# PKU-EPIC/HOTrack

Measured on AMD Instinct MI355X. Metric: HandTrackNet point-cloud frames/sec (N=1024), higher is better.
Workload: dtype f32; 1 GPU; HandTrackNet forward, batch=64 synthetic 1024-pt clouds per GPU (BASELINE configs[1]); per_gpu_batch=64, global_batch=64, npoints=1024, parallelism=dp1 (independent batches, no collective), world_size=1, resident_batches_rotated=5, dead_attention_elided=True, fused_sa_kernels=True, launch=hipGraph replay, batches_in_flight=4, hip_hw_queues=4, sa_compute_units=256, weights=deterministic random init (no checkpoint available offline)

## Files before the change

### hotrack_amd/csrc/row_chain.hip

```cpp
#include "pn2_common.h"
#include "../../include/pn2_ext.h"

namespace pn2 {
namespace rchain {

typedef float f32x4 __attribute__((ext_vector_type(4)));

constexpr int CH = 128, CC = 384, CQ = 512;
constexpr int KX = 144;
constexpr int XQ = 33;
constexpr int LDX = 152, LDH = 136, LDC = 392;
constexpr int MAXB = 1024;
constexpr int GROUP_COST_SMALL = 31, GROUP_COST_LARGE = 20;

struct ChainArgs {
    int B, N, ldx, ldo;
    const float *x;
    const int *list, *counts;
    const float *wa, *ba, *wb, *bb, *wc, *bc, *wq;
    float *out;
};

template <int NT, int MT, int KG, int LD>
__device__ __forceinline__ void mm(f32x4 (&acc)[NT][MT], const float *__restrict__ wp, const float *xs, int lane) {
    const f32x4 *w4 = reinterpret_cast<const f32x4 *>(wp) + lane;
    const float *xr = xs + (lane & 15) * LD + 4 * (lane >> 4);
    f32x4 w[2][NT], x[2][MT];
    auto load = [&](int kg, int slot) {
#pragma unroll
        for (int nt = 0; nt < NT; ++nt) w[slot][nt] = w4[(nt * KG + kg) * 64];
#pragma unroll
        for (int mt = 0; mt < MT; ++mt) x[slot][mt] = *reinterpret_cast<const f32x4 *>(xr + mt * 16 * LD + 16 * kg);
    };
    auto step = [&](int slot) {
#pragma unroll
        for (int s = 0; s < 4; ++s)
#pragma unroll
            for (int nt = 0; nt < NT; ++nt)
#pragma unroll
                for (int mt = 0; mt < MT; ++mt)
                    acc[nt][mt] = __builtin_amdgcn_mfma_f32_16x16x4f32(w[slot][nt][s], x[slot][mt][s], acc[nt][mt], 0, 0, 0);
    };
    load(0, 0);
    int kg = 0;
#pragma unroll 1
    for (; kg + 2 <= KG; kg += 2) {
        load(kg + 1, 1);
        step(0);
        if (kg + 2 < KG) load(kg + 2, 0);
        step(1);
    }
    if constexpr (KG & 1) step(0);
}

template <int NT, int MT>
__device__ __forceinline__ void init_bias(f32x4 (&acc)[NT][MT], const float *__restrict__ bias, int nt0, int lane) {
#pragma unroll
    for (int nt = 0; nt < NT; ++nt) {
        const f32x4 b = *reinterpret_cast<const f32x4 *>(bias + (nt0 + nt) * 16 + 4 * (lane >> 4));
#pragma unroll
        for (int mt = 0; mt < MT; ++mt) acc[nt][mt] = b;
    }
}

template <int NT, int MT>
__device__ __forceinline__ void relu_to_lds(const f32x4 (&acc)[NT][MT], float *dst, int ld, int nt0, int lane) {
#pragma unroll
    for (int nt = 0; nt < NT; ++nt)
#pragma unroll
        for (int mt = 0; mt < MT; ++mt) {
            const f32x4 v = acc[nt][mt];
            *reinterpret_cast<f32x4 *>(dst + (mt * 16 + (lane & 15)) * ld + (nt0 + nt) * 16 + 4 * (lane >> 4)) =
                (f32x4){fmaxf(v.x, 0.f), fmaxf(v.y, 0.f), fmaxf(v.z, 0.f), fmaxf(v.w, 0.f)};
        }
}

struct Smem {
    int *rows;
    int *p_small;
    int *p_large;
    float *r1;
    float *r2;
};

__device__ __forceinline__ int lookup(const ChainArgs &A, const Smem &S, int seq, int e) {
    const int *P = seq ? S.p_large : S.p_small;
    int lo = 0, hi = A.B;
    while (hi - lo > 1) {
        const int mid = (lo + hi) >> 1;
        if (P[mid] <= e) lo = mid; else hi = mid;
    }
    const int off = seq ? (S.p_small[lo + 1] - S.p_small[lo]) : 0;
    return lo * A.N + A.list[(size_t)lo * A.N + off + (e - P[lo])];
}

template <int MT>
__device__ void tile(const ChainArgs &A, const Smem &S, int seq, int e0, int cnt) {
    const int tid = (int)threadIdx.x, lane = tid & 63, w = tid >> 6;
    constexpr int R = MT * 16;
    if (tid < R) S.rows[tid] = tid < cnt ? lookup(A, S, seq, e0 + tid) : -1;
    __syncthreads();
    for (int i = tid; i < R * (KX / 4); i += 256) {
        const int r = i / (KX / 4), q = i - r * (KX / 4);
        const int g = S.rows[r];
        f32x4 v = {0.f, 0.f, 0.f, 0.f};
        if (g >= 0 && q < XQ) {
            v = *reinterpret_cast<const f32x4 *>(A.x + (size_t)g * A.ldx + 4 * q);
            if (q == XQ - 1) v.w = 0.f;
        }
        *reinterpret_cast<f32x4 *>(S.r1 + r * LDX + 4 * q) = v;
    }
    __syncthreads();
    {
        f32x4 acc[2][MT];
        init_bias(acc, A.ba, 2 * w, lane);
        mm<2, MT, KX / 16, LDX>(acc, A.wa + (size_t)(2 * w) * (KX / 16) * 256, S.r1, lane);
        relu_to_lds(acc, S.r2, LDH, 2 * w, lane);
    }
    __syncthreads();
    {
        f32x4 acc[2][MT];
        init_bias(acc, A.bb, 2 * w, lane);
        mm<2, MT, CH / 16, LDH>(acc, A.wb + (size_t)(2 * w) * (CH / 16) * 256, S.r2, lane);
        relu_to_lds(acc, S.r1, LDH, 2 * w, lane);
    }
    __syncthreads();
#pragma unroll 1
    for (int p = 0; p < 2; ++p) {
// ... 185 lines not shown
```

### hotrack_amd/ext.py

```python
from __future__ import annotations

import ctypes
import os

import torch

from . import pointnet2_hip as _native

_lib = _native._lib
_vp, _ci = ctypes.c_void_p, ctypes.c_int
_lib.pn2x_kabsch.argtypes = [_ci, _ci, _ci, _vp, _vp, _vp, _vp, _vp]
_lib.pn2x_kabsch.restype = _ci


def kabsch(x: torch.Tensor, y: torch.Tensor):
    x = x.float().contiguous()
    y = y.float().contiguous()
    if x.dim() == 2:
        x = x.unsqueeze(0)
    B, num, _ = y.shape
    xb = x.shape[0]
    if xb not in (1, B) or x.shape[1] != num:
        raise ValueError(f"kabsch: x {tuple(x.shape)} does not match y {tuple(y.shape)}")
    px = _native._ptr(x, "x", torch.float32, xb * num * 3)
# ... 616 lines not shown


def row_lists(gi: torch.Tensor, gi_small, n: int):
    if gi.dim() != 3 or gi.dtype != torch.int32 or not gi.is_cuda:
        raise TypeError("row_lists: gi must be a (B,J,K) int32 GPU tensor")
    gi = gi.contiguous()
    B, J, KL = gi.shape
    if gi_small is not None:
        if gi_small.dim() != 3 or gi_small.shape[:2] != (B, J) or gi_small.dtype != torch.int32 or gi_small.device != gi.device:
            raise ValueError("row_lists: gi_small must be (B,J,K2) int32 on gi's device")
        gi_small = gi_small.contiguous()
    KS = gi_small.shape[2] if gi_small is not None else KL
    lst = torch.empty((B, n), dtype=torch.int32, device=gi.device)
    counts = torch.empty((B, 2), dtype=torch.int32, device=gi.device)
    with torch.cuda.device(gi.device):
        _native._check(_native._call(_lib.pn2x_row_lists, "row_lists_kernel", None, B, n, J, KL, KS, gi.data_ptr(),
                                     None if gi_small is None else gi_small.data_ptr(), lst.data_ptr(), counts.data_ptr(),
                                     _native._stream(gi)), "row_lists")
    return lst, counts


def row_chain_supported(c_in: int, c_h: int, c_conv: int, c_q: int) -> bool:
    return bool(_lib.pn2x_row_chain_supported(c_in, c_h, c_conv, c_q))


def row_chain_pack(W: torch.Tensor) -> torch.Tensor:
    n_out, k = W.shape
    kp = (k + 15) // 16 * 16
    Wp = torch.zeros((n_out, kp), dtype=torch.float32, device=W.device)
    Wp[:, :k] = W
    return Wp.view(n_out // 16, 16, kp // 16, 4, 4).permute(0, 2, 3, 1, 4).contiguous()


def row_chain(x: torch.Tensor, lst: torch.Tensor, counts: torch.Tensor, wa, ba, wb, bb, wc, bc, wq, out: torch.Tensor = None,
              grid: int = 0) -> torch.Tensor:
    if x.dim() != 3 or not x.is_cuda or x.dtype != torch.float32 or x.stride(2) != 1 or x.stride(0) != x.shape[1] * x.stride(1):
        raise TypeError("row_chain: x must be a (B,N,C) float32 GPU tensor with contiguous rows")
    B, N, _ = x.shape
    f32 = torch.float32
    if out is None:
        out = torch.empty((B, N, 512), dtype=f32, device=x.device)
    if out.shape[:2] != (B, N) or out.shape[2] < 512 or out.stride(2) != 1 or out.stride(0) != N * out.stride(1) or out.dtype != f32:
        raise ValueError("row_chain: out must be (B,N,>=512) float32 with contiguous rows")
    if lst.shape != (B, N) or counts.shape != (B, 2) or lst.dtype != torch.int32 or counts.dtype != torch.int32:
        raise ValueError("row_chain: list (B,N) / counts (B,2) int32 from row_lists")
    with torch.cuda.device(x.device):
        _native._check(_native._call(_lib.pn2x_row_chain, "row_chain_kernel", None, B, N, x.data_ptr(), x.stride(1), lst.data_ptr(),
                                     counts.data_ptr(), _native._ptr(wa, "wa", f32, 128 * 144), _native._ptr(ba, "ba", f32, 128),
                                     _native._ptr(wb, "wb", f32, 128 * 128), _native._ptr(bb, "bb", f32, 128),
                                     _native._ptr(wc, "wc", f32, 384 * 128), _native._ptr(bc, "bc", f32, 384),
                                     _native._ptr(wq, "wq", f32, 512 * 384), out.data_ptr(), out.stride(1), int(grid),
                                     _native._stream(x)), "row_chain")
    return out
```

### include/pn2_ext.h

```cpp
#ifndef PN2_EXT_H
#define PN2_EXT_H

#include "pn2_hip.h"

#ifdef __cplusplus
extern "C" {
#endif

int pn2x_kabsch(int b, int xb, int num, const float *x, const float *y, float *R, float *t, void *stream);
int pn2x_kabsch_backward(int b, int xb, int num, const float *x, const float *y, const float *R, const float *grad_R,
                         const float *grad_t, float *grad_y, void *stream);

int pn2x_hand_frame(int b, int xb, int num, int n, int j, const float *palm_template, const float *kp,
                    const int *palm_idx, const float *points, float scale, float *R, float *t, float *xyz2,
                    float *xyz1, float *xyz2_copy, int copy_ld, int *nonfinite, void *stream);

int pn2x_sa_mlp_max(int b, int n, int s, int k, int c1, int c2, int c3, const float *a1f, int a1f_ld,
                    const float *xyz, const float *cxyz, const float *wx, const float *b1, const float *cadd,
                    int cadd_ld, const int *idx,
                    const float *w2, const float *b2, const float *w3, const float *b3, float *out,
                    long out_b, int out_s, int out_c, void *stream);
int pn2x_sa_mlp_max_supported(int k, int c1, int c2, int c3);

int pn2x_bias_act(int b, int c, int n, float *y, const float *bias, int relu, void *stream);
// ... 18 lines not shown
int pn2x_fps_prefix_flags(int n);
int pn2x_furthest_point_sampling_prefix(int b, int n, int m, const float *xyz, const int *flags, int nflags, int *idx, void *stream);

int pn2x_knn_indices(int b, int n, int m, int k, int k2, const float *unknown, const float *known, int *idx, int *idx2, void *stream);

int pn2x_ball_query_picks(int b, int n, int m, float radius, int nsample, const float *xyz, const int *picks, float *new_xyz,
                          int *idx, float *new_xyz_copy, int copy_ld, void *stream);

long pn2x_ball_query_grid_scratch_words(int b, int n);
int pn2x_ball_query_grid(int b, int n, int m, float radius, int nsample, const float *new_xyz, const float *xyz, int *idx,
                         void *scratch, long scratch_words, void *stream);

int pn2x_gather_rows(int b, int n, int m, int c, const float *src, const int *idx, float *out, void *stream);

int pn2x_bias_act_pm(long rows, int c, float *y, int ldy, const float *bias, long rows_per_bias, int relu, void *stream);

int pn2x_max_rows(int b, int r, int c, const float *x, float *out, void *stream);

int pn2x_copy_multi_max(void);
int pn2x_copy_multi(int n, void *const *dst, const void *const *src, const long *bytes, void *stream);

int pn2x_add_layernorm(long rows, int c, const float *x, const float *y, const float *bias, const float *g1,
                       const float *b1, float eps1, const float *g2, const float *b2, float eps2, float *out, void *stream);

int pn2x_pose_head(int b, int j, int c, const float *h, const float *w, const float *bias, const float *xyz1,
                   const float *R, const float *t, float scale, float *kp_hand, float *kp_cam, const int *nonfinite,
                   void *stream);

typedef struct pn2x_sa_problem {
    int n, s, k;
    const float *a1f;
    int a1f_ld;
    const float *xyz, *cxyz, *wx, *b1, *cadd;
    int cadd_ld;
    const int *idx;
    const float *w2, *b2, *w3, *b3;
    float *out;
    long out_b;
    int out_s, out_c;
} pn2x_sa_problem;
int pn2x_sa_set_compute_units(int n);
int pn2x_mlp2_rows_supported(int c1, int c2, int c3);
int pn2x_mlp2_rows(long rows, int c1, int c2, int c3, const float *x, int ldx, const float *w2, const float *w2e, const float *b2,
                   const float *w3, const float *b3, float *out, int ldo, void *stream);
int pn2x_sa_mlp_max_pair_supported(int k0, int k1, int c1, int c2, int c3);
int pn2x_sa_mlp_max_pair(int b, int c1, int c2, int c3, const pn2x_sa_problem *p0, const pn2x_sa_problem *p1, void *stream);

int pn2x_row_lists(int b, int n, int j, int k_large, int k_small, const int *gi, const int *gi_small, int *list, int *counts,
                   void *stream);
int pn2x_row_chain_supported(int c_in, int c_h, int c_conv, int c_q);
int pn2x_row_chain(int b, int n, const float *x, int ldx, const int *list, const int *counts, const float *wa, const float *ba,
                   const float *wb, const float *bb, const float *wc, const float *bc, const float *wq, float *out, int ldo,
                   int grid, void *stream);

int pn2x_bn_sums_doubles(int c);
int pn2x_bn_stats(long rows, int c, const float *y, int ldy, double *sums, void *stream);
int pn2x_bn_relu_apply(long rows, int c, const float *y, int ldy, const double *sums, const float *gamma, const float *beta,
                       const float *conv_bias, float eps, float momentum, float *running_mean, float *running_var,
                       long long *num_batches_tracked, float *save_mean, float *save_invstd, float *h, int ldh, int relu,
                       void *stream);
int pn2x_bn_relu_bwd(long rows, int c, const float *dh, int ldd, const float *y, int ldy, const float *mean,
                     const float *invstd, const float *gamma, const float *beta, int relu, double *sums, float *dy, int ldo,
                     float *dgamma, float *dbeta, float *dbias, void *stream);
int pn2x_sa_layer1(int b, int n, int s, int k, int c1, const float *a1f, int a1f_ld, const float *xyz, const float *cxyz,
                   const float *wx, int wx_ld, const float *cadd, int cadd_ld, const int *idx, float *out, float *rel_out,
                   void *stream);
int pn2x_sa_layer1_stats(int b, int n, int s, int k, int c1, const float *a1f, int a1f_ld, const float *xyz, const float *cxyz,
                         const float *wx, int wx_ld, const float *cadd, int cadd_ld, const int *idx, float *out, float *rel_out,
                         double *sums, void *stream);
int pn2x_sa_layer1_stats_pair(int b, int n, int s, const float *xyz, const float *cxyz, int k_a, int c1_a, const float *a1f_a, int a1f_ld_a,
                              const float *wx_a, int wx_ld_a, const float *cadd_a, int cadd_ld_a, const int *idx_a, float *out_a,
                              float *rel_out_a, double *sums_a, int k_b, int c1_b, const float *a1f_b, int a1f_ld_b, const float *wx_b,
                              int wx_ld_b, const float *cadd_b, int cadd_ld_b, const int *idx_b, float *out_b, float *rel_out_b,
                              double *sums_b, void *stream);
int pn2x_scatter_add_rows(int b, int n, int m, int c, const float *dout, int ldo, const int *idx, float *din, int ldi,
                          void *stream);
int pn2x_three_interpolate_pm_grad(int b, int c, int m, int n, const float *dout, int ldo, const int *idx,
                                   const float *weight, float *dpoints, int ldp, void *stream);

int pn2x_inverse_index(int b, int n_dst, int l, const int *idx, int *offsets, int *order, void *stream);
int pn2x_rows_segment_sum(int b, int n_dst, int m_src, int t, int c, const float *dout, int ldo, const int *offsets,
                          const int *order, const float *weight, float *din, int ldi, int accumulate, void *stream);
int pn2x_rows_segment_sum_pair(int b, int n_dst, int m_a, int c_a, const float *dout_a, int ldo_a, const int *offsets_a, const int *order_a,
                               float *din_a, int ldi_a, int m_b, int c_b, const float *dout_b, int ldo_b, const int *offsets_b,
                               const int *order_b, float *din_b, int ldi_b, int accumulate, void *stream);

long pn2x_scatter_cm_scratch_ints(int t, int b, int n_dst, int m_src);
int pn2x_scatter_cm(int t, int b, int c, int n_dst, int m_src, const float *grad_out, const int *idx, const float *weight,
                    float *grad_points, int *scratch, long scratch_ints, void *stream);

int pn2x_bn_relu_max(long groups, int k, int c, const float *y, int ldy, const double *sums, const float *gamma, const float *beta,
                     const float *conv_bias, float eps, float momentum, float *running_mean, float *running_var,
                     long long *num_batches_tracked, float *save_mean, float *save_invstd, float *out, int *arg, void *stream);
int pn2x_bn_relu_max_ld(long groups, int k, int c, const float *y, int ldy, const double *sums, const float *gamma, const float *beta,
                        const float *conv_bias, float eps, float momentum, float *running_mean, float *running_var,
                        long long *num_batches_tracked, float *save_mean, float *save_invstd, float *out, int ldo, int *arg, void *stream);
int pn2x_bn_relu_max_pair(long groups_a, int k_a, int c_a, const float *y_a, int ldy_a, const double *sums_a, const float *gamma_a,
                          const float *beta_a, const float *conv_bias_a, float eps_a, float momentum_a, float *running_mean_a,
                          float *running_var_a, long long *nbt_a, float *save_mean_a, float *save_invstd_a, float *out_a, int ldo_a,
                          int *arg_a, long groups_b, int k_b, int c_b, const float *y_b, int ldy_b, const double *sums_b,
                          const float *gamma_b, const float *beta_b, const float *conv_bias_b, float eps_b, float momentum_b,
                          float *running_mean_b, float *running_var_b, long long *nbt_b, float *save_mean_b, float *save_invstd_b,
                          float *out_b, int ldo_b, int *arg_b, void *stream);
int pn2x_bn_relu_max_bwd(long groups, int k, int c, const float *dout, const int *arg, const float *y, int ldy, const float *mean,
                         const float *invstd, const float *gamma, const float *beta, double *sums, float *dy, int ldo, float *dgamma,
                         float *dbeta, float *dbias, void *stream);
// ... 126 lines not shown
```

### network/models/fast_eval.py

```python
from __future__ import annotations

import torch
import torch.nn.functional as F



def _lin_relu(x2d: torch.Tensor, W: torch.Tensor, b: torch.Tensor) -> torch.Tensor:
    from hotrack_amd import ext
    return ext.linear(x2d, W, b, relu=True)


def _lin(x2d: torch.Tensor, W: torch.Tensor, b: torch.Tensor = None) -> torch.Tensor:
    from hotrack_amd import ext
    return ext.linear(x2d, W, b)


class FastEval:
    MAX_POINTS = 16384

    def __init__(self, net):
        self.net = net
        self._shapes_seen = set()
        self._key = None
        self.P = None
# ... 57 lines not shown
        gemm_tuning.enable()
        net, bh = self.net, self.net.bhand
        P = {}

        def msg(mod, i):
            return [fold(c, n) for c, n in zip(mod.conv_blocks[i], mod.bn_blocks[i])]

        (W1, b1), l2, l3 = msg(bh.sa1, 0)
        P["sa1"] = dict(wx=W1.contiguous(), b1=b1, l2=l2, l3=l3)
        (W1, b1), l2, l3 = msg(bh.sa2, 0)
        D = W1.shape[1] - 3
        P["sa2"] = dict(w1f=W1[:, :D].contiguous(), wx=W1[:, D:].contiguous(), b1=b1, l2=l2, l3=l3)
        sa3 = [fold(c, n) for c, n in zip(bh.sa3.mlp_convs, bh.sa3.mlp_bns)]
        W = sa3[0][0]
        sa3[0] = (torch.cat([W[:, 3:], W[:, :3]], dim=1).contiguous(), sa3[0][1])
        P["sa3"] = sa3
        fp3 = [fold(c, n) for c, n in zip(bh.fp3.mlp_convs, bh.fp3.mlp_bns)]
        c_l2 = bh.sa2.out_channel
        P["fp3"] = dict(wa=fp3[0][0][:, :c_l2].contiguous(), wb=fp3[0][0][:, c_l2:].contiguous(), b=fp3[0][1], rest=fp3[1:])
        P["fp2"] = [fold(c, n) for c, n in zip(bh.fp2.mlp_convs, bh.fp2.mlp_bns)]
        fp1 = [fold(c, n) for c, n in zip(bh.fp1.mlp_convs, bh.fp1.mlp_bns)]
        W = fp1[0][0]
        fp1[0] = (torch.cat([W[:, 3:], W[:, :3]], dim=1).contiguous(), fp1[0][1])
        P["fp1"] = fp1
        import os
        from hotrack_amd import ext
        P["fp1_fused"] = None
        c_in = fp1[0][0].shape[1] - 3
        if os.environ.get("HOTRACK_MLP2", "1") != "0" and len(fp1) == 2 and c_in == P["fp2"][-1][0].shape[0] and ext.mlp2_rows_supported(c_in, fp1[0][0].shape[0], fp1[1][0].shape[0]):
            P["fp1_fused"] = dict(w2=fp1[0][0][:, :c_in].contiguous(), w2e=fp1[0][0][:, c_in:].contiguous(), b2=fp1[0][1],
                                  w3=fp1[1][0].contiguous(), b3=fp1[1][1])
        P["conv1"] = fold(bh.conv1, bh.bn1)
        C = bh.out_dim
        wq, q = [], {}
        for name, mod in (("q1", net.q1), ("q2", net.q2)):
            for i in range(2):
                (W1, b1), l2, l3 = msg(mod, i)
                wq.append(W1[:, :C])
                q[(name, i)] = dict(wx=W1[:, C:C + 3].contiguous(), b1=b1, l2=l2, l3=l3, K=mod.nsample_list[i],
                                    wc=W1[:, C + 3:] if W1.shape[1] > C + 3 else None)
        P["q"] = q
        Ks = [q[("q1", i)]["K"] for i in range(2)]
        i_s = Ks.index(min(Ks))
        P["wq_order"] = (i_s, 1 - i_s)
        P["wq"] = torch.cat([torch.cat([wq[i], wq[2 + i]], dim=0) for i in P["wq_order"]], dim=0)
        P["row_chain"] = None
        Wc = P["conv1"][0]
        if (len(fp1) == 2 and c_in == P["fp2"][-1][0].shape[0] and Ks[0] != Ks[1] and fp1[0][0].shape[1] == c_in + 3
                and ext.row_chain_supported(c_in, fp1[0][0].shape[0], Wc.shape[0], 4 * wq[0].shape[0])
                and fp1[1][0].shape == (c_in, c_in) and Wc.shape[1] == c_in and C == Wc.shape[0]):
            P["row_chain"] = dict(wa=ext.row_chain_pack(fp1[0][0]), ba=fp1[0][1].contiguous(),
                                  wb=ext.row_chain_pack(fp1[1][0]), bb=fp1[1][1].contiguous(),
                                  wc=ext.row_chain_pack(Wc), bc=P["conv1"][1].contiguous(), wq=ext.row_chain_pack(P["wq"]))
        P["wc2"] = torch.cat([q[("q2", 0)]["wc"], q[("q2", 1)]["wc"]], dim=0).contiguous()
        P["head_w"] = net.final_mlp[2].weight.detach().squeeze(-1).contiguous()
        P["r1"] = (net.r1.linear.weight.detach().squeeze(-1), net.r1.linear.bias.detach(), net.r1._perm.t().contiguous())
        P["r2"] = (net.r2.linear.weight.detach().squeeze(-1), net.r2.linear.bias.detach(), net.r2._perm.t().contiguous())
        self.P, self._key = P, key
        return P

    def _perm_idx(self, perm, B):
        key = ("perm", B, str(perm.device))
        if key not in self._idents:
            self._idents[key] = perm.reshape(1, -1).to(torch.int32).expand(B, -1).contiguous()
        return self._idents[key]

    @staticmethod
    def _q_scales(ext, name, plan, q, xyz1, c1q, a_col, cadd, out, c_q):
        probs = []
        for i, (idx, a, nb_xyz) in enumerate(plan):
            p = q[(name, i)]
            probs.append(dict(idx=idx, w2=p["l2"][0], b2=p["l2"][1], w3=p["l3"][0], b3=p["l3"][1], a1f=a[:, :, a_col:a_col + c1q],
                              xyz=nb_xyz, cxyz=xyz1, wx=p["wx"], b1=p["b1"],
                              cadd=None if cadd is None else cadd[:, :, i * c1q:(i + 1) * c1q], out=out[:, :, i * c_q:(i + 1) * c_q]))
        if len(probs) == 2:
            ext.sa_mlp_max_pair(*probs)
        else:
            for p in probs:
                ext.sa_mlp_max(p.pop("idx"), p.pop("w2"), p.pop("b2"), p.pop("w3"), p.pop("b3"), **p)

    def forward(self, input, flag_dict):
        from hotrack_amd import gemm_tuning
        shape = tuple(input["hand_points"].shape[:2])
        first = shape not in self._shapes_seen
        self._shapes_seen.add(shape)
        with gemm_tuning.scope(tune=first):
            return self._forward(input, flag_dict)

    def _forward(self, input, flag_dict):
        G = self._geometry(input, flag_dict)
        return None if G is None else self._dense(G, flag_dict)

    def _geometry(self, input, flag_dict):
        from hotrack_amd import ext
        net = self.net
        P = self.prepare()
        if P is None:
            return None
        dev = net.device
        if flag_dict["track_flag"]:
            palm = input["pred_palm_template"]
        else:
            palm = input["gt_hand_pose"]["palm_template"]
        palm = palm.to(dev).float()
        kp = input["jittered_hand_kp"].to(dev).float()
        pts = input["hand_points"].to(dev).float()
        B, N, _ = pts.shape
        J = kp.shape[1]
        f32 = dict(dtype=torch.float32, device=pts.device)

        if net.handframe != "kp":
            raise NotImplementedError("fast path covers handframe='kp' (HandTrackNet's configuration)")
        if kp.shape[1] != 21:
            raise NotImplementedError("fast path covers the 21-keypoint hand")
        palm_idx = self._palm_idx(pts.device)
        c_i = P["fp2"][-1][0].shape[0]
        fp1_in = torch.empty((B, N, c_i + 4), **f32)
        nonfinite = torch.empty(B, dtype=torch.int32, device=pts.device)
        R, t, xyz2, xyz1 = ext.hand_frame(palm.contiguous(), kp.contiguous(), palm_idx, pts.contiguous(), 0.2,
                                          xyz2_copy=fp1_in[:, :, c_i:c_i + 3], nonfinite=nonfinite)
        scale = self._scale(pts.device)
        canon = {"scale": scale, "rotation": R, "translation": t}
        tt = t.transpose(1, 2)

        bh = net.bhand
        p = P["sa1"]
        S1, K1 = bh.sa1.npoint, bh.sa1.nsample_list[0]
        qK = [P["q"][("q1", i)]["K"] for i in range(2)]
        knn_req = (xyz1, max(qK), min(qK) if min(qK) < max(qK) else 0)
        _, l1_xyz, i_l2, idx1, knn_lists = ext.fps_two_level(xyz2, S1, bh.sa2.npoint, query=(bh.sa1.radius_list[0], K1), knn=knn_req)
        return dict(P=P, pts=pts, B=B, N=N, J=J, c_i=c_i, fp1_in=fp1_in, nonfinite=nonfinite, R=R, t=t, xyz2=xyz2, xyz1=xyz1,
                    canon=canon, S1=S1, K1=K1, l1_xyz=l1_xyz, i_l2=i_l2, idx1=idx1, knn_lists=knn_lists)

    def _dense(self, G, flag_dict):
        from hotrack_amd import ext
        from hotrack_amd import pointnet2_utils as ops
        net, bh = self.net, self.net.bhand
        P, pts, B, N, J, c_i, fp1_in, nonfinite = G["P"], G["pts"], G["B"], G["N"], G["J"], G["c_i"], G["fp1_in"], G["nonfinite"]
        R, t, xyz2, xyz1, canon, S1, K1 = G["R"], G["t"], G["xyz2"], G["xyz1"], G["canon"], G["S1"], G["K1"]
        l1_xyz, i_l2, idx1, knn_lists = G["l1_xyz"], G["i_l2"], G["idx1"], G["knn_lists"]
        f32 = dict(dtype=torch.float32, device=pts.device)
        dev = net.device
        p = P["sa1"]
        c_l1 = p["l3"][0].shape[0]
        fp2_w = P["fp2"][0][0].shape[1]
        fp2_in = torch.empty((B, S1, fp2_w), **f32)
        l1_feat = fp2_in[:, :, :c_l1]
        ext.sa_mlp_max(idx1, *p["l2"], *p["l3"], xyz=xyz2, cxyz=l1_xyz, wx=p["wx"], b1=p["b1"], out=l1_feat)

        p = P["sa2"]
        S2, K2 = bh.sa2.npoint, bh.sa2.nsample_list[0]
        c_l2 = p["l3"][0].shape[0]
        sa3_in = torch.empty((B, S2, c_l2 + 4), **f32)
        idx2, l2_xyz = ext.ball_query_picks(bh.sa2.radius_list[0], K2, l1_xyz, i_l2, xyz_copy=sa3_in[:, :, c_l2:c_l2 + 3])
        a1f = _lin(l1_feat.reshape(B * S1, c_l1), p["w1f"]).view(B, S1, -1)
        l2_feat = sa3_in[:, :, :c_l2]
        ext.sa_mlp_max(idx2, *p["l2"], *p["l3"], a1f=a1f, xyz=l1_xyz, cxyz=l2_xyz, wx=p["wx"], b1=p["b1"], out=l2_feat)

        x = sa3_in.view(B * S2, c_l2 + 4)[:, :c_l2 + 3]
        for W, b in P["sa3"]:
            x = _lin_relu(x, W, b)
        l3 = ext.max_rows(x.view(B, S2, -1))

        p = P["fp3"]
        g = _lin(l3, p["wb"], p["b"])
        if B == 1:
            h = _lin_relu(sa3_in.view(S2, c_l2 + 4)[:, :c_l2], p["wa"], g.view(-1)).view(B, S2, -1)
        else:
            h = _lin(sa3_in.view(B * S2, c_l2 + 4)[:, :c_l2], p["wa"]).view(B, S2, -1)
            ext.bias_act_pm_(h, g, rows_per_bias=S2, relu=True)
        x = h.view(B * S2, -1)
        for W, b in p["rest"]:
            x = _lin_relu(x, W, b)
        l2_out = x.view(B, S2, -1)

        ext.three_nn_interpolate_pm(l1_xyz, l2_xyz, l2_out, fp2_in[:, :, c_l1:])
        x = fp2_in.view(B * S1, fp2_w)
        for W, b in P["fp2"]:
            x = _lin_relu(x, W, b)
        l1_out = x.view(B, S1, -1)

        assert c_i == l1_out.shape[2]
        ext.three_nn_interpolate_pm(xyz2, l1_xyz, l1_out, fp1_in[:, :, :c_i])
        q = P["q"]
        Ks = [q[("q1", i)]["K"] for i in range(2)]
        kmin, kmax = min(Ks), max(Ks)
        gi, gi_small = knn_lists
        c_q = q[("q1", 0)]["l3"][0].shape[0]
        c1q = q[("q1", 0)]["l2"][0].shape[1]
        rc = P["row_chain"]
        if self.row_chain and rc is not None and B * N >= 32768 and B <= ext.ROW_CHAIN_MAX_B and gi_small is not None:
            lst, counts = ext.row_lists(gi, gi_small, N)
            a_all = torch.empty((B, N, 4 * c1q), **f32)
            ext.row_chain(fp1_in, lst, counts, rc["wa"], rc["ba"], rc["wb"], rc["bb"], rc["wc"], rc["bc"], rc["wq"], out=a_all)
        else:
            f = P["fp1_fused"]
            if f is not None:
                x = ext.mlp2_rows(fp1_in.view(B * N, c_i + 4), f["w2"], f["b2"], f["w3"], f["b3"], w2e=f["w2e"])
            else:
                x = fp1_in.view(B * N, c_i + 4)[:, :c_i + 3]
                for W, b in P["fp1"]:
                    x = _lin_relu(x, W, b)
            src2 = _lin_relu(x, *P["conv1"])
            a_all = _lin(src2, P["wq"]).view(B, N, -1)
        plan = []
        for i, K in enumerate(Ks):
            j = P["wq_order"].index(i)
            idx = gi if K == kmax else (gi_small if K == kmin and gi_small is not None else gi[:, :, :K].contiguous())
            plan.append((idx, a_all[:, :, 2 * c1q * j:2 * c1q * (j + 1)], xyz2))
        f11 = torch.empty((B, J, 2 * c_q), **f32)
        self._q_scales(ext, "q1", plan, q, xyz1, c1q, 0, None, f11, c_q)
        Wr, br, perm = P["r1"]
        f12 = _lin(ext.gather_rows(f11, self._perm_idx(perm, B)).view(B * J, -1), Wr, br)
        cadd = _lin(f12, P["wc2"]).view(B, J, -1)
        f13 = torch.empty((B, J, 2 * c_q), **f32)
        self._q_scales(ext, "q2", plan, q, xyz1, c1q, c1q, cadd, f13, c_q)
        Wr, br, perm = P["r2"]
        f14 = _lin(ext.gather_rows(f13, self._perm_idx(perm, B)).view(B * J, -1), Wr, br)

        s11, c11, c3 = net.transt.s11, net.transt.c11, net.c3
        wf, bf = net.final_mlp[0].weight.squeeze(-1), net.final_mlp[0].bias
        if ext.ln_linear_supported(f14.shape[0], f14.shape[1]):
            x, hdn = ext.ln_linear(f14, s11.norm1, c11.linear1.weight, c11.linear1.bias, relu=True, ln2=c11.norm1)
            y = _lin(hdn, c11.linear2.weight)
            x, hdn = ext.ln_linear(x, c11.norm2, c3.linear1.weight, c3.linear1.bias, relu=True, y=y, ybias=c11.linear2.bias, ln2=c3.norm1)
            y = _lin(hdn, c3.linear2.weight)
            x, hdn = ext.ln_linear(x, c3.norm2, wf, bf, relu=True, y=y, ybias=c3.linear2.bias)
        else:
            x = ext.add_layernorm(f14, s11.norm1, ln2=c11.norm1)
            for blk, nxt in ((c11, c3.norm1), (c3, None)):
                hdn = _lin_relu(x, blk.linear1.weight, blk.linear1.bias)
                x = ext.add_layernorm(x, blk.norm2, y=_lin(hdn, blk.linear2.weight), bias=blk.linear2.bias, ln2=nxt)
            hdn = _lin_relu(x, wf, bf)
        pred_hf, pred_kp = ext.pose_head(hdn, P["head_w"], net.final_mlp[2].bias, xyz1, R, t, 0.2, nonfinite=nonfinite)

        ret = {"canon_pose": canon}
        ret["pred_kp_handframe"] = pred_hf.transpose(1, 2)
        ret["init_kp_handframe"] = xyz1.transpose(1, 2)
        ret["points_handframe"] = xyz2.transpose(1, 2)
        ret["pred_kp"] = pred_kp
        if flag_dict.get("IKNet_flag", False):
            d4, _ = ops.knn(4, ret["pred_kp"].contiguous(), pts.contiguous())
            d4 = d4.mean(dim=-1)
            d4[:, 0] -= 0.01
# ... 4 lines not shown
```

Baseline: 84860 frames/s.

## Fuse SA3 MLP+max and FP3 MLP chains into two MFMA row-chain kernels

```diff
diff --git a/hotrack_amd/csrc/mfma_rows.h b/hotrack_amd/csrc/mfma_rows.h
--- /dev/null
+++ b/hotrack_amd/csrc/mfma_rows.h
@@ -0,0 +1,64 @@
+#pragma once
+#include <hip/hip_runtime.h>
+
+namespace pn2 {
+namespace mrows {
+
+typedef float f32x4 __attribute__((ext_vector_type(4)));
+
+template <int NT, int MT, int KG, int LD>
+__device__ __forceinline__ void mm(f32x4 (&acc)[NT][MT], const float *__restrict__ wp, const float *xs, int lane) {
+    const f32x4 *w4 = reinterpret_cast<const f32x4 *>(wp) + lane;
+    const float *xr = xs + (lane & 15) * LD + 4 * (lane >> 4);
+    f32x4 w[2][NT], x[2][MT];
+    auto load = [&](int kg, int slot) {
+#pragma unroll
+        for (int nt = 0; nt < NT; ++nt) w[slot][nt] = w4[(nt * KG + kg) * 64];
+#pragma unroll
+        for (int mt = 0; mt < MT; ++mt) x[slot][mt] = *reinterpret_cast<const f32x4 *>(xr + mt * 16 * LD + 16 * kg);
+    };
+    auto step = [&](int slot) {
+#pragma unroll
+        for (int s = 0; s < 4; ++s)
+#pragma unroll
+            for (int nt = 0; nt < NT; ++nt)
+#pragma unroll
+                for (int mt = 0; mt < MT; ++mt)
+                    acc[nt][mt] = __builtin_amdgcn_mfma_f32_16x16x4f32(w[slot][nt][s], x[slot][mt][s], acc[nt][mt], 0, 0, 0);
+    };
+    load(0, 0);
+    int kg = 0;
+#pragma unroll 1
+    for (; kg + 2 <= KG; kg += 2) {
+        load(kg + 1, 1);
+        step(0);
+        if (kg + 2 < KG) load(kg + 2, 0);
+        step(1);
+    }
+    if constexpr (KG & 1) step(0);
+}
+
+template <int NT, int MT>
+__device__ __forceinline__ void init_bias(f32x4 (&acc)[NT][MT], const float *__restrict__ bias, int nt0, int lane) {
+#pragma unroll
+    for (int nt = 0; nt < NT; ++nt) {
+        const f32x4 b = *reinterpret_cast<const f32x4 *>(bias + (nt0 + nt) * 16 + 4 * (lane >> 4));
+#pragma unroll
+        for (int mt = 0; mt < MT; ++mt) acc[nt][mt] = b;
+    }
+}
+
+template <int NT, int MT>
+__device__ __forceinline__ void relu_to_lds(const f32x4 (&acc)[NT][MT], float *dst, int ld, int nt0, int lane) {
+#pragma unroll
+    for (int nt = 0; nt < NT; ++nt)
+#pragma unroll
+        for (int mt = 0; mt < MT; ++mt) {
+            const f32x4 v = acc[nt][mt];
+            *reinterpret_cast<f32x4 *>(dst + (mt * 16 + (lane & 15)) * ld + (nt0 + nt) * 16 + 4 * (lane >> 4)) =
+                (f32x4){fmaxf(v.x, 0.f), fmaxf(v.y, 0.f), fmaxf(v.z, 0.f), fmaxf(v.w, 0.f)};
+        }
+}
+
+}
+}
diff --git a/hotrack_amd/csrc/mid_chain.hip b/hotrack_amd/csrc/mid_chain.hip
--- /dev/null
+++ b/hotrack_amd/csrc/mid_chain.hip
@@ -0,0 +1,195 @@
+#include "pn2_common.h"
+#include "mfma_rows.h"
+#include "../../include/pn2_ext.h"
+
+namespace pn2 {
+namespace mchain {
+
+using mrows::f32x4;
+using mrows::init_bias;
+using mrows::mm;
+using mrows::relu_to_lds;
+
+constexpr int MT = 2, TR = 16 * MT;
+constexpr int CL2 = 128, CL3 = 512;
+constexpr int C1 = 128, C2 = 128;
+constexpr int CF = 256;
+constexpr int KX = 144;
+constexpr int XQ = 33;
+constexpr int LDX = 152, LDH = 136, LDF = 264;
+
+constexpr size_t SA3_LDS = (size_t)TR * (LDX + LDH) * sizeof(float);
+constexpr size_t FP3_LDS = (size_t)(TR * (LDH + LDF) + CL3 + 4 * CF + CF) * sizeof(float);
+
+__device__ __forceinline__ float row16_max(float v) {
+    PN2_DPP_STEP("v_max_f32_dpp", v, "quad_perm:[1,0,3,2] row_mask:0xf bank_mask:0xf");
+    PN2_DPP_STEP("v_max_f32_dpp", v, "quad_perm:[2,3,0,1] row_mask:0xf bank_mask:0xf");
+    PN2_DPP_STEP("v_max_f32_dpp", v, "row_half_mirror row_mask:0xf bank_mask:0xf");
+    PN2_DPP_STEP("v_max_f32_dpp", v, "row_mirror row_mask:0xf bank_mask:0xf");
+    return v;
+}
+
+__global__ __launch_bounds__(256) void sa3_chain_kernel(const float *__restrict__ x, int ldx, const float *__restrict__ w1,
+                                                        const float *__restrict__ b1, const float *__restrict__ w2,
+                                                        const float *__restrict__ b2, const float *__restrict__ w3,
+                                                        const float *__restrict__ b3, float *__restrict__ part) {
+    extern __shared__ __attribute__((aligned(16))) float smem[];
+    float *r1 = smem, *r2 = smem + TR * LDX;
+    const int tid = (int)threadIdx.x, lane = tid & 63, w = tid >> 6;
+    const size_t row0 = (size_t)blockIdx.x * TR;
+    for (int i = tid; i < TR * (KX / 4); i += 256) {
+        const int r = i / (KX / 4), q = i - r * (KX / 4);
+        f32x4 v = {0.f, 0.f, 0.f, 0.f};
+        if (q < XQ) {
+            v = *reinterpret_cast<const f32x4 *>(x + (row0 + r) * ldx + 4 * q);
+            if (q == XQ - 1) v.w = 0.f;
+        }
+        *reinterpret_cast<f32x4 *>(r1 + r * LDX + 4 * q) = v;
+    }
+    __syncthreads();
+    {
+        f32x4 acc[2][MT];
+        init_bias(acc, b1, 2 * w, lane);
+        mm<2, MT, KX / 16, LDX>(acc, w1 + (size_t)(2 * w) * (KX / 16) * 256, r1, lane);
+        relu_to_lds(acc, r2, LDH, 2 * w, lane);
+    }
+    __syncthreads();
+    {
+        f32x4 acc[2][MT];
+        init_bias(acc, b2, 2 * w, lane);
+        mm<2, MT, C1 / 16, LDH>(acc, w2 + (size_t)(2 * w) * (C1 / 16) * 256, r2, lane);
+        relu_to_lds(acc, r1, LDH, 2 * w, lane);
+    }
+    __syncthreads();
+    float *dst = part + (size_t)blockIdx.x * CL3 + 4 * (lane >> 4);
+#pragma unroll 1
+    for (int p = 0; p < 2; ++p) {
+        const int nt0 = (p * 4 + w) * 4;
+        f32x4 acc[4][MT];
+        init_bias(acc, b3, nt0, lane);
+        mm<4, MT, C2 / 16, LDH>(acc, w3 + (size_t)nt0 * (C2 / 16) * 256, r1, lane);
+#pragma unroll
+        for (int nt = 0; nt < 4; ++nt) {
+            f32x4 m = acc[nt][0];
+#pragma unroll
+            for (int mt = 1; mt < MT; ++mt)
+                m = (f32x4){fmaxf(m.x, acc[nt][mt].x), fmaxf(m.y, acc[nt][mt].y), fmaxf(m.z, acc[nt][mt].z), fmaxf(m.w, acc[nt][mt].w)};
+            m = (f32x4){fmaxf(row16_max(m.x), 0.f), fmaxf(row16_max(m.y), 0.f), fmaxf(row16_max(m.z), 0.f), fmaxf(row16_max(m.w), 0.f)};
+            if ((lane & 15) == 0) *reinterpret_cast<f32x4 *>(dst + (nt0 + nt) * 16) = m;
+        }
+    }
+}
+
+__global__ __launch_bounds__(256) void fp3_chain_kernel(int s, const float *__restrict__ x, int ldx, const float *__restrict__ part,
+                                                        const float *__restrict__ wgt, const float *__restrict__ bg,
+                                                        const float *__restrict__ wa, const float *__restrict__ wf,
+                                                        const float *__restrict__ bf, float *__restrict__ out, int ldo) {
+    extern __shared__ __attribute__((aligned(16))) float smem[];
+    float *r1 = smem, *r2 = r1 + TR * LDH, *l3 = r2 + TR * LDF, *gp = l3 + CL3, *g = gp + 4 * CF;
+    const int tid = (int)threadIdx.x, lane = tid & 63, w = tid >> 6;
+    const size_t row0 = (size_t)blockIdx.x * TR;
+    const int np = s / TR;
+    const int b = (int)(row0 / (size_t)s);
+    for (int i = tid; i < TR * (CL2 / 4); i += 256) {
+        const int r = i / (CL2 / 4), q = i - r * (CL2 / 4);
+        *reinterpret_cast<f32x4 *>(r1 + r * LDH + 4 * q) = *reinterpret_cast<const f32x4 *>(x + (row0 + r) * ldx + 4 * q);
+    }
+    for (int k = tid; k < CL3; k += 256) {
+        const float *pp = part + (size_t)b * np * CL3 + k;
+        float m = pp[0];
+        for (int i = 1; i < np; ++i) m = fmaxf(m, pp[(size_t)i * CL3]);
+        l3[k] = m;
+    }
+    __syncthreads();
+    {
+        const int q = tid & 63, kq = tid >> 6;
+        const f32x4 *wt = reinterpret_cast<const f32x4 *>(wgt) + (size_t)(kq * (CL3 / 4)) * 64 + q;
+        const float *lk = l3 + kq * (CL3 / 4);
+        f32x4 a = {0.f, 0.f, 0.f, 0.f};
+#pragma unroll 8
+        for (int k = 0; k < CL3 / 4; ++k) a = __builtin_elementwise_fma(wt[(size_t)k * 64], (f32x4)lk[k], a);
+        *reinterpret_cast<f32x4 *>(gp + kq * CF + 4 * q) = a;
+    }
+    __syncthreads();
+    if (tid < CF / 4) {
+        const f32x4 *g4 = reinterpret_cast<const f32x4 *>(gp) + tid;
+        *reinterpret_cast<f32x4 *>(g + 4 * tid) =
+            *reinterpret_cast<const f32x4 *>(bg + 4 * tid) + ((g4[0] + g4[CF / 4]) + (g4[2 * CF / 4] + g4[3 * CF / 4]));
+    }
+    __syncthreads();
+    const int nt0 = 4 * w;
+    {
+        f32x4 acc[4][MT];
+        init_bias(acc, g, nt0, lane);
+        mm<4, MT, CL2 / 16, LDH>(acc, wa + (size_t)nt0 * (CL2 / 16) * 256, r1, lane);
+        relu_to_lds(acc, r2, LDF, nt0, lane);
+    }
+    __syncthreads();
+    {
+        f32x4 acc[4][MT];
+        init_bias(acc, bf, nt0, lane);
+        mm<4, MT, CF / 16, LDF>(acc, wf + (size_t)nt0 * (CF / 16) * 256, r2, lane);
+#pragma unroll
+        for (int mt = 0; mt < MT; ++mt) {
+            float *o = out + (row0 + mt * 16 + (lane & 15)) * ldo + nt0 * 16 + 4 * (lane >> 4);
+#pragma unroll
+            for (int nt = 0; nt < 4; ++nt) {
+                const f32x4 v = acc[nt][mt];
+                *reinterpret_cast<f32x4 *>(o + nt * 16) = (f32x4){fmaxf(v.x, 0.f), fmaxf(v.y, 0.f), fmaxf(v.z, 0.f), fmaxf(v.w, 0.f)};
+            }
+        }
+    }
+}
+
+inline bool misaligned16(std::initializer_list<const void *> ps) {
+    uintptr_t u = 0;
+    for (const void *p : ps) u |= (uintptr_t)p;
+    return u % 16 != 0;
+}
+
+}
+}
+
+extern "C" int pn2x_sa3_chain_supported(int s, int c_in, int c1, int c2, int c3) {
+    using namespace pn2::mchain;
+    return (s > 0 && s % TR == 0 && c_in == CL2 && c1 == C1 && c2 == C2 && c3 == CL3) ? 1 : 0;
+}
+
+extern "C" int pn2x_sa3_chain(int b, int s, const float *x, int ldx, const float *w1, const float *b1, const float *w2,
+                              const float *b2, const float *w3, const float *b3, float *part, void *stream) {
+    using namespace pn2;
+    using namespace pn2::mchain;
+    if (b < 0 || s < 1 || s % TR || ldx < XQ * 4 || ldx % 4) return PN2_EINVAL;
+    if ((long)b * s >= (1L << 31)) return PN2_ERANGE;
+    if (b == 0) return PN2_OK;
+    if (!x || !w1 || !b1 || !w2 || !b2 || !w3 || !b3 || !part) return PN2_ENULL;
+    if (misaligned16({x, w1, b1, w2, b2, w3, b3, part})) return PN2_EINVAL;
+    static PerDeviceOnce raised;
+    if (raised.first_use())
+        (void)hipFuncSetAttribute((const void *)sa3_chain_kernel, hipFuncAttributeMaxDynamicSharedMemorySize, (int)SA3_LDS);
+    hipLaunchKernelGGL(sa3_chain_kernel, dim3((unsigned)((long)b * s / TR)), dim3(256), SA3_LDS, (hipStream_t)stream, x, ldx, w1,
+                       b1, w2, b2, w3, b3, part);
+    return check_launch();
+}
+
+extern "C" int pn2x_fp3_chain_supported(int s, int c_l2, int c_l3, int c1, int c2) {
+    using namespace pn2::mchain;
+    return (s > 0 && s % TR == 0 && c_l2 == CL2 && c_l3 == CL3 && c1 == CF && c2 == CF) ? 1 : 0;
+}
+
+extern "C" int pn2x_fp3_chain(int b, int s, const float *x, int ldx, const float *part, const float *wgt, const float *bg,
+                              const float *wa, const float *wf, const float *bf, float *out, int ldo, void *stream) {
+    using namespace pn2;
+    using namespace pn2::mchain;
+    if (b < 0 || s < 1 || s % TR || ldx < CL2 || ldx % 4 || ldo < CF || ldo % 4) return PN2_EINVAL;
+    if ((long)b * s >= (1L << 31)) return PN2_ERANGE;
+    if (b == 0) return PN2_OK;
+    if (!x || !part || !wgt || !bg || !wa || !wf || !bf || !out) return PN2_ENULL;
+    if (misaligned16({x, part, wgt, bg, wa, wf, bf, out})) return PN2_EINVAL;
+    static PerDeviceOnce raised;
+    if (raised.first_use())
+        (void)hipFuncSetAttribute((const void *)fp3_chain_kernel, hipFuncAttributeMaxDynamicSharedMemorySize, (int)FP3_LDS);
+    hipLaunchKernelGGL(fp3_chain_kernel, dim3((unsigned)((long)b * s / TR)), dim3(256), FP3_LDS, (hipStream_t)stream, s, x, ldx,
+                       part, wgt, bg, wa, wf, bf, out, ldo);
+    return check_launch();
+}
diff --git a/hotrack_amd/csrc/row_chain.hip b/hotrack_amd/csrc/row_chain.hip
--- a/hotrack_amd/csrc/row_chain.hip
+++ b/hotrack_amd/csrc/row_chain.hip
@@ -1,10 +1,14 @@
 #include "pn2_common.h"
+#include "mfma_rows.h"
 #include "../../include/pn2_ext.h"
 
 namespace pn2 {
 namespace rchain {
 
-typedef float f32x4 __attribute__((ext_vector_type(4)));
+using mrows::f32x4;
+using mrows::init_bias;
+using mrows::mm;
+using mrows::relu_to_lds;
 
 constexpr int CH = 128, CC = 384, CQ = 512;
 constexpr int KX = 144;
@@ -20,60 +24,6 @@
     const float *wa, *ba, *wb, *bb, *wc, *bc, *wq;
     float *out;
 };
-
-template <int NT, int MT, int KG, int LD>
-__device__ __forceinline__ void mm(f32x4 (&acc)[NT][MT], const float *__restrict__ wp, const float *xs, int lane) {
-    const f32x4 *w4 = reinterpret_cast<const f32x4 *>(wp) + lane;
-    const float *xr = xs + (lane & 15) * LD + 4 * (lane >> 4);
-    f32x4 w[2][NT], x[2][MT];
-    auto load = [&](int kg, int slot) {
-#pragma unroll
-        for (int nt = 0; nt < NT; ++nt) w[slot][nt] = w4[(nt * KG + kg) * 64];
-#pragma unroll
-        for (int mt = 0; mt < MT; ++mt) x[slot][mt] = *reinterpret_cast<const f32x4 *>(xr + mt * 16 * LD + 16 * kg);
-    };
-    auto step = [&](int slot) {
-#pragma unroll
-        for (int s = 0; s < 4; ++s)
-#pragma unroll
-            for (int nt = 0; nt < NT; ++nt)
-#pragma unroll
-                for (int mt = 0; mt < MT; ++mt)
-                    acc[nt][mt] = __builtin_amdgcn_mfma_f32_16x16x4f32(w[slot][nt][s], x[slot][mt][s], acc[nt][mt], 0, 0, 0);
-    };
-    load(0, 0);
-    int kg = 0;
-#pragma unroll 1
-    for (; kg + 2 <= KG; kg += 2) {
-        load(kg + 1, 1);
-        step(0);
-        if (kg + 2 < KG) load(kg + 2, 0);
-        step(1);
-    }
-    if constexpr (KG & 1) step(0);
-}
-
-template <int NT, int MT>
-__device__ __forceinline__ void init_bias(f32x4 (&acc)[NT][MT], const float *__restrict__ bias, int nt0, int lane) {
-#pragma unroll
-    for (int nt = 0; nt < NT; ++nt) {
-        const f32x4 b = *reinterpret_cast<const f32x4 *>(bias + (nt0 + nt) * 16 + 4 * (lane >> 4));
-#pragma unroll
-        for (int mt = 0; mt < MT; ++mt) acc[nt][mt] = b;
-    }
-}
-
-template <int NT, int MT>
-__device__ __forceinline__ void relu_to_lds(const f32x4 (&acc)[NT][MT], float *dst, int ld, int nt0, int lane) {
-#pragma unroll
-    for (int nt = 0; nt < NT; ++nt)
-#pragma unroll
-        for (int mt = 0; mt < MT; ++mt) {
-            const f32x4 v = acc[nt][mt];
-            *reinterpret_cast<f32x4 *>(dst + (mt * 16 + (lane & 15)) * ld + (nt0 + nt) * 16 + 4 * (lane >> 4)) =
-                (f32x4){fmaxf(v.x, 0.f), fmaxf(v.y, 0.f), fmaxf(v.z, 0.f), fmaxf(v.w, 0.f)};
-        }
-}
 
 struct Smem {
     int *rows;
diff --git a/hotrack_amd/ext.py b/hotrack_amd/ext.py
--- a/hotrack_amd/ext.py
+++ b/hotrack_amd/ext.py
@@ -692,3 +692,71 @@
                                      _native._ptr(wq, "wq", f32, 512 * 384), out.data_ptr(), out.stride(1), int(grid),
                                      _native._stream(x)), "row_chain")
     return out
+
+
+_lib.pn2x_sa3_chain_supported.argtypes = [_ci] * 5
+_lib.pn2x_sa3_chain_supported.restype = _ci
+_lib.pn2x_sa3_chain.argtypes = [_ci, _ci, _vp, _ci] + [_vp] * 7 + [_vp]
+_lib.pn2x_sa3_chain.restype = _ci
+_lib.pn2x_fp3_chain_supported.argtypes = [_ci] * 5
+_lib.pn2x_fp3_chain_supported.restype = _ci
+_lib.pn2x_fp3_chain.argtypes = [_ci, _ci, _vp, _ci] + [_vp] * 6 + [_vp, _ci, _vp]
+_lib.pn2x_fp3_chain.restype = _ci
+MID_CHAIN_TILE = 32
+
+
+def sa3_chain_supported(s: int, c_in: int, c1: int, c2: int, c3: int) -> bool:
+    return bool(_lib.pn2x_sa3_chain_supported(s, c_in, c1, c2, c3))
+
+
+def fp3_chain_supported(s: int, c_l2: int, c_l3: int, c1: int, c2: int) -> bool:
+    return bool(_lib.pn2x_fp3_chain_supported(s, c_l2, c_l3, c1, c2))
+
+
+def _chain_rows(x: torch.Tensor, name: str, min_cols: int):
+    if x.dim() != 3 or not x.is_cuda or x.dtype != torch.float32 or x.stride(2) != 1 or x.shape[2] < min_cols or \
+            x.stride(0) != x.shape[1] * x.stride(1):
+        raise TypeError(f"{name}: expected a (B,S,>={min_cols}) float32 GPU tensor with contiguous rows, got {tuple(x.shape)} {x.stride()}")
+    return x.shape[0], x.shape[1]
+
+
+def sa3_chain(x: torch.Tensor, w1, b1, w2, b2, w3, b3, part: torch.Tensor = None) -> torch.Tensor:
+    B, S = _chain_rows(x, "sa3_chain", 132)
+    T = MID_CHAIN_TILE
+    if S % T:
+        raise ValueError(f"sa3_chain: S = {S} is not a multiple of {T}")
+    f32 = torch.float32
+    if part is None:
+        part = torch.empty((B, S // T, 512), dtype=f32, device=x.device)
+    if tuple(part.shape) != (B, S // T, 512) or not part.is_contiguous() or part.dtype != f32:
+        raise ValueError(f"sa3_chain: part must be a contiguous (B, S/{T}, 512) float32 tensor")
+    with torch.cuda.device(x.device):
+        _native._check(_native._call(_lib.pn2x_sa3_chain, "sa3_chain_kernel", None, B, S, x.data_ptr(), x.stride(1),
+                                     _native._ptr(w1, "w1", f32, 128 * 144), _native._ptr(b1, "b1", f32, 128),
+                                     _native._ptr(w2, "w2", f32, 128 * 128), _native._ptr(b2, "b2", f32, 128),
+                                     _native._ptr(w3, "w3", f32, 512 * 128), _native._ptr(b3, "b3", f32, 512), part.data_ptr(),
+                                     _native._stream(x)), "sa3_chain")
+    return part
+
+
+def fp3_chain(x: torch.Tensor, part: torch.Tensor, wgt, bg, wa, wf, bf, out: torch.Tensor = None) -> torch.Tensor:
+    B, S = _chain_rows(x, "fp3_chain", 128)
+    T = MID_CHAIN_TILE
+    if S % T:
+        raise ValueError(f"fp3_chain: S = {S} is not a multiple of {T}")
+    f32 = torch.float32
+    if out is None:
+        out = torch.empty((B, S, 256), dtype=f32, device=x.device)
+    _chain_rows(out, "fp3_chain: out", 256)
+    if out.shape[:2] != (B, S):
+        raise ValueError("fp3_chain: out must be (B,S,>=256)")
+    if tuple(part.shape) != (B, S // T, 512) or not part.is_contiguous() or part.dtype != f32:
+        raise ValueError(f"fp3_chain: part must be a contiguous (B, S/{T}, 512) float32 tensor")
+    if tuple(wgt.shape) != (512, 256):
+        raise ValueError("fp3_chain: wgt must be Wg^T, (512, 256)")
+    with torch.cuda.device(x.device):
+        _native._check(_native._call(_lib.pn2x_fp3_chain, "fp3_chain_kernel", None, B, S, x.data_ptr(), x.stride(1), part.data_ptr(),
+                                     _native._ptr(wgt, "wgt", f32, 512 * 256), _native._ptr(bg, "bg", f32, 256),
+                                     _native._ptr(wa, "wa", f32, 256 * 128), _native._ptr(wf, "wf", f32, 256 * 256),
+                                     _native._ptr(bf, "bf", f32, 256), out.data_ptr(), out.stride(1), _native._stream(x)), "fp3_chain")
+    return out
diff --git a/include/pn2_ext.h b/include/pn2_ext.h
--- a/include/pn2_ext.h
+++ b/include/pn2_ext.h
@@ -94,6 +94,13 @@
 int pn2x_row_chain(int b, int n, const float *x, int ldx, const int *list, const int *counts, const float *wa, const float *ba,
                    const float *wb, const float *bb, const float *wc, const float *bc, const float *wq, float *out, int ldo,
                    int grid, void *stream);
+
+int pn2x_sa3_chain_supported(int s, int c_in, int c1, int c2, int c3);
+int pn2x_sa3_chain(int b, int s, const float *x, int ldx, const float *w1, const float *b1, const float *w2, const float *b2,
+                   const float *w3, const float *b3, float *part, void *stream);
+int pn2x_fp3_chain_supported(int s, int c_l2, int c_l3, int c1, int c2);
+int pn2x_fp3_chain(int b, int s, const float *x, int ldx, const float *part, const float *wgt, const float *bg, const float *wa,
+                   const float *wf, const float *bf, float *out, int ldo, void *stream);
 
 int pn2x_bn_sums_doubles(int c);
 int pn2x_bn_stats(long rows, int c, const float *y, int ldy, double *sums, void *stream);
diff --git a/network/models/fast_eval.py b/network/models/fast_eval.py
--- a/network/models/fast_eval.py
+++ b/network/models/fast_eval.py
@@ -133,12 +133,27 @@
             P["row_chain"] = dict(wa=ext.row_chain_pack(fp1[0][0]), ba=fp1[0][1].contiguous(),
                                   wb=ext.row_chain_pack(fp1[1][0]), bb=fp1[1][1].contiguous(),
                                   wc=ext.row_chain_pack(Wc), bc=P["conv1"][1].contiguous(), wq=ext.row_chain_pack(P["wq"]))
+        P["mid_chain"] = None
+        S2 = bh.sa2.npoint
+        pf = P["fp3"]
+        if (len(sa3) == 3 and len(pf["rest"]) == 1 and sa3[0][0].shape[1] == c_l2 + 3
+                and ext.sa3_chain_supported(S2, c_l2, sa3[0][0].shape[0], sa3[1][0].shape[0], sa3[2][0].shape[0])
+                and sa3[1][0].shape[1] == sa3[0][0].shape[0] and sa3[2][0].shape[1] == sa3[1][0].shape[0]
+                and ext.fp3_chain_supported(S2, pf["wa"].shape[1], pf["wb"].shape[1], pf["wa"].shape[0], pf["rest"][0][0].shape[0])
+                and pf["wb"].shape[1] == sa3[2][0].shape[0] and pf["rest"][0][0].shape[1] == pf["wa"].shape[0]):
+            P["mid_chain"] = dict(sa3=[t for W, b in sa3 for t in (ext.row_chain_pack(W), b.contiguous())],
+                                  wgt=pf["wb"].t().contiguous(), bg=pf["b"].contiguous(), wa=ext.row_chain_pack(pf["wa"]),
+                                  wf=ext.row_chain_pack(pf["rest"][0][0]), bf=pf["rest"][0][1].contiguous())
         P["wc2"] = torch.cat([q[("q2", 0)]["wc"], q[("q2", 1)]["wc"]], dim=0).contiguous()
         P["head_w"] = net.final_mlp[2].weight.detach().squeeze(-1).contiguous()
         P["r1"] = (net.r1.linear.weight.detach().squeeze(-1), net.r1.linear.bias.detach(), net.r1._perm.t().contiguous())
         P["r2"] = (net.r2.linear.weight.detach().squeeze(-1), net.r2.linear.bias.detach(), net.r2._perm.t().contiguous())
         self.P, self._key = P, key
         return P
+
+    def _large_batch(self, B, N) -> bool:
+        from hotrack_amd import ext
+        return self.row_chain and B * N >= 32768 and B <= ext.ROW_CHAIN_MAX_B
 
     def _perm_idx(self, perm, B):
         key = ("perm", B, str(perm.device))
@@ -238,22 +253,28 @@
         l2_feat = sa3_in[:, :, :c_l2]
         ext.sa_mlp_max(idx2, *p["l2"], *p["l3"], a1f=a1f, xyz=l1_xyz, cxyz=l2_xyz, wx=p["wx"], b1=p["b1"], out=l2_feat)
 
-        x = sa3_in.view(B * S2, c_l2 + 4)[:, :c_l2 + 3]
-        for W, b in P["sa3"]:
-            x = _lin_relu(x, W, b)
-        l3 = ext.max_rows(x.view(B, S2, -1))
-
-        p = P["fp3"]
-        g = _lin(l3, p["wb"], p["b"])
-        if B == 1:
-            h = _lin_relu(sa3_in.view(S2, c_l2 + 4)[:, :c_l2], p["wa"], g.view(-1)).view(B, S2, -1)
-        else:
-            h = _lin(sa3_in.view(B * S2, c_l2 + 4)[:, :c_l2], p["wa"]).view(B, S2, -1)
-            ext.bias_act_pm_(h, g, rows_per_bias=S2, relu=True)
-        x = h.view(B * S2, -1)
-        for W, b in p["rest"]:
-            x = _lin_relu(x, W, b)
-        l2_out = x.view(B, S2, -1)
+        large = self._large_batch(B, N)
+        mc = P["mid_chain"]
+        if large and mc is not None:
+            part = ext.sa3_chain(sa3_in, *mc["sa3"])
+            l2_out = ext.fp3_chain(sa3_in, part, mc["wgt"], mc["bg"], mc["wa"], mc["wf"], mc["bf"])
+        else:
+            x = sa3_in.view(B * S2, c_l2 + 4)[:, :c_l2 + 3]
+            for W, b in P["sa3"]:
+                x = _lin_relu(x, W, b)
+            l3 = ext.max_rows(x.view(B, S2, -1))
+
+            p = P["fp3"]
+            g = _lin(l3, p["wb"], p["b"])
+            if B == 1:
+                h = _lin_relu(sa3_in.view(S2, c_l2 + 4)[:, :c_l2], p["wa"], g.view(-1)).view(B, S2, -1)
+            else:
+                h = _lin(sa3_in.view(B * S2, c_l2 + 4)[:, :c_l2], p["wa"]).view(B, S2, -1)
+                ext.bias_act_pm_(h, g, rows_per_bias=S2, relu=True)
+            x = h.view(B * S2, -1)
+            for W, b in p["rest"]:
+                x = _lin_relu(x, W, b)
+            l2_out = x.view(B, S2, -1)
 
         ext.three_nn_interpolate_pm(l1_xyz, l2_xyz, l2_out, fp2_in[:, :, c_l1:])
         x = fp2_in.view(B * S1, fp2_w)
@@ -270,7 +291,7 @@
         c_q = q[("q1", 0)]["l3"][0].shape[0]
         c1q = q[("q1", 0)]["l2"][0].shape[1]
         rc = P["row_chain"]
-        if self.row_chain and rc is not None and B * N >= 32768 and B <= ext.ROW_CHAIN_MAX_B and gi_small is not None:
+        if large and rc is not None and gi_small is not None:
             lst, counts = ext.row_lists(gi, gi_small, N)
             a_all = torch.empty((B, N, 4 * c1q), **f32)
             ext.row_chain(fp1_in, lst, counts, rc["wa"], rc["ba"], rc["wb"], rc["bb"], rc["wc"], rc["bc"], rc["wq"], out=a_all)
```

New measurement: 87880 frames/s (median of 6 runs). +3.6%, better.
